# GeoStat-Framework/PyKrige

Measured on NVIDIA H100. Metric: kriged grid points/sec (N data -> M grid), higher is better.
Workload: dtype f64

## Files before the change

include/krige_b200.h:

```cpp
#ifndef KRIGE_B200_H
#define KRIGE_B200_H

#include <stddef.h>
#include <stdint.h>

#ifdef __cplusplus
extern "C" {
#endif

#define KB200_OK            0
#define KB200_EBADARG      -1
#define KB200_EUNSUPPORTED -2
#define KB200_ESINGULAR    -3
#define KB200_ECUDA        -4
#define KB200_ENOMEM       -5
#define KB200_ESTATE       -6

#define KB200_VG_LINEAR       0
#define KB200_VG_POWER        1
#define KB200_VG_GAUSSIAN     2
#define KB200_VG_EXPONENTIAL  3
#define KB200_VG_SPHERICAL    4
#define KB200_VG_HOLE_EFFECT  5
#define KB200_VG_TABLE        6
// ... 97 lines not shown
                            int exact_values, double eps,
                            int n_rl, int n_hd, const double* drift_data);
int kb200_group_set_problem_knn(kb200_group g, int dim, int64_t n,
                                const double* x, const double* y, const double* z,
                                const double* values,
                                const double* center, const double* aniso,
                                int model, const double* vparams, int n_vparams,
                                int exact_values, double eps);
int kb200_group_execute_points(kb200_group g, int64_t m,
                               const double* px, const double* py, const double* pz,
                               const double* drift_pts,
                               double* z_out, double* ss_out);
int kb200_group_execute_grid(kb200_group g,
                             int64_t nx, int64_t ny, int64_t nz,
                             const double* gx, const double* gy, const double* gz,
                             const double* drift_pts,
                             int64_t first, int64_t count,
                             double* z_out, double* ss_out);
int kb200_group_execute_knn_points(kb200_group g, int k, int64_t m,
                                   const double* px, const double* py, const double* pz,
                                   double* z_out, double* ss_out);
int kb200_group_execute_knn_grid(kb200_group g, int k,
                                 int64_t nx, int64_t ny, int64_t nz,
                                 const double* gx, const double* gy, const double* gz,
                                 int64_t first, int64_t count,
                                 double* z_out, double* ss_out);

int kb200_set_coordinates(kb200_handle h, int coordinates_type);

int kb200_set_stream(kb200_handle h, void* cuda_stream);

int  kb200_last_timings(kb200_handle h, double* ms, int n);
void kb200_reset_counters(kb200_handle h);

int kb200_set_variogram_table(kb200_handle h, int64_t n_nodes, double dmax, const double* gamma_nodes);

int kb200_set_pseudo_inverse(kb200_handle h, int enable);

int kb200_set_values(kb200_handle h, int n_fields, int64_t n, const double* values);

int kb200_experimental_variogram(kb200_handle h, int dim, int64_t n,
                                 const double* x, const double* y, const double* z, const double* values,
                                 int nlags, double* counts, double* lag_sum, double* semi_sum, double* dminmax);

int kb200_statistics(kb200_handle h, double* delta, double* sigma);

int kb200_loo(kb200_handle h, double* z, double* sigmasq);
int kb200_knn_loo(kb200_handle h, int k, double* z, double* sigmasq);

int kb200_lgo(kb200_handle h, const int32_t* group, int n_groups, double* z, double* sigmasq);
int kb200_knn_lgo(kb200_handle h, int k, const int32_t* group, int n_groups, double* z, double* sigmasq);

int64_t kb200_debug_fetch(kb200_handle h, int what, double* out, int64_t cap);

#ifdef __cplusplus
}
#endif
#endif
```

pykrige_b200/_cabi.py:

```python
import ctypes
import os
import numpy as np

_HERE = os.path.dirname(os.path.abspath(__file__))
LIB_PATH = os.path.join(_HERE, "libkrige_b200.so")

KB200_OK = 0
KB200_EBADARG = -1
KB200_EUNSUPPORTED = -2
KB200_ESINGULAR = -3
KB200_ECUDA = -4
KB200_ENOMEM = -5
KB200_ESTATE = -6

KB200_F64 = 0
KB200_F32 = 1
KB200_F64X = 2
KB200_F64X5 = 3
KB200_F64X4 = 4
DTYPES = {"float64": KB200_F64, "float32": KB200_F32, "float64x": KB200_F64X, "float64x5": KB200_F64X5,
          "float64x4": KB200_F64X4}
MAX_DRIFT = 15
MAX_FIELDS = 64

EXPORTS = [
    "kb200_create", "kb200_destroy", "kb200_last_error", "kb200_version",
    "kb200_set_problem", "kb200_execute_points", "kb200_execute_grid",
    "kb200_execute_points_dev", "kb200_execute_grid_dev",
    "kb200_execute_knn_points", "kb200_execute_knn_grid", "kb200_execute_knn_grid_dev",
    "kb200_set_problem_knn",
    "kb200_blob_bytes", "kb200_blob_ptr", "kb200_describe_problem", "kb200_blob_commit",
    "kb200_set_coordinates", "kb200_set_stream", "kb200_last_timings", "kb200_reset_counters", "kb200_debug_fetch",
    "kb200_experimental_variogram", "kb200_statistics", "kb200_loo", "kb200_knn_loo", "kb200_lgo", "kb200_knn_lgo",
    "kb200_set_pseudo_inverse",
    "kb200_set_variogram_table", "kb200_set_device_drift", "kb200_set_values",
    "kb200_group_create", "kb200_group_destroy", "kb200_group_last_error", "kb200_group_size", "kb200_group_member",
    "kb200_group_set_problem", "kb200_group_set_problem_knn", "kb200_group_execute_points",
    "kb200_group_execute_grid", "kb200_group_execute_knn_points", "kb200_group_execute_knn_grid",
]

_c_double_p = ctypes.POINTER(ctypes.c_double)
_lib = None


class KrigeB200Error(RuntimeError):
    pass


def load_library():
    global _lib
    if _lib is not None:
        return _lib
    if not os.path.exists(LIB_PATH):
        raise KrigeB200Error(
            "libkrige_b200.so is not built (%s). Run `python -c 'import __graft_entry__ as g; g.build()'` "
            "or `make -C pykrige_b200/csrc`. backend='cuda' has no CPU fallback." % LIB_PATH
        )
    lib = ctypes.CDLL(LIB_PATH)
    h = ctypes.c_void_p
    i64 = ctypes.c_int64
    i32 = ctypes.c_int
    dp = ctypes.c_void_p
    lib.kb200_create.argtypes = [ctypes.POINTER(h), i32]
    lib.kb200_destroy.argtypes = [h]
    lib.kb200_destroy.restype = None
    lib.kb200_last_error.argtypes = [h]
    lib.kb200_last_error.restype = ctypes.c_char_p
    lib.kb200_version.restype = i32
    prob = [h, i32, i32, i64, dp, dp, dp, dp, dp, dp, i32, dp, i32, i32, ctypes.c_double, i32, i32, dp]
    lib.kb200_set_problem.argtypes = prob
    lib.kb200_describe_problem.argtypes = prob
    lib.kb200_set_problem_knn.argtypes = [h, i32, i64, dp, dp, dp, dp, dp, dp, i32, dp, i32, i32, ctypes.c_double]
    lib.kb200_execute_points.argtypes = [h, i64, dp, dp, dp, dp, dp, dp]
    lib.kb200_execute_points_dev.argtypes = [h, i64, dp, dp, dp, dp, dp, dp]
    grid = [h, i64, i64, i64, dp, dp, dp, dp, i64, i64, dp, dp]
    lib.kb200_execute_grid.argtypes = grid
    lib.kb200_execute_grid_dev.argtypes = grid
    lib.kb200_execute_knn_points.argtypes = [h, i32, i64, dp, dp, dp, dp, dp]
    kgrid = [h, i32, i64, i64, i64, dp, dp, dp, i64, i64, dp, dp]
    lib.kb200_execute_knn_grid.argtypes = kgrid
    lib.kb200_execute_knn_grid_dev.argtypes = kgrid
    lib.kb200_blob_bytes.argtypes = [h]
    lib.kb200_blob_bytes.restype = i64
    lib.kb200_blob_ptr.argtypes = [h]
    lib.kb200_blob_ptr.restype = ctypes.c_void_p
    lib.kb200_blob_commit.argtypes = [h]
    lib.kb200_set_coordinates.argtypes = [h, i32]
    lib.kb200_set_stream.argtypes = [h, ctypes.c_void_p]
    lib.kb200_last_timings.argtypes = [h, _c_double_p, i32]
    lib.kb200_reset_counters.argtypes = [h]
    lib.kb200_reset_counters.restype = None
    lib.kb200_debug_fetch.argtypes = [h, i32, dp, i64]
    lib.kb200_debug_fetch.restype = i64
    lib.kb200_experimental_variogram.argtypes = [h, i32, i64, dp, dp, dp, dp, i32, dp, dp, dp, dp]
    lib.kb200_statistics.argtypes = [h, dp, dp]
    lib.kb200_loo.argtypes = [h, dp, dp]
    lib.kb200_knn_loo.argtypes = [h, i32, dp, dp]
    lib.kb200_lgo.argtypes = [h, dp, i32, dp, dp]
    lib.kb200_knn_lgo.argtypes = [h, i32, dp, i32, dp, dp]
    lib.kb200_set_pseudo_inverse.argtypes = [h, i32]
    lib.kb200_set_variogram_table.argtypes = [h, i64, ctypes.c_double, dp]
    lib.kb200_set_device_drift.argtypes = [h, i32, dp, i64, i64, dp, dp, dp]
    lib.kb200_set_values.argtypes = [h, i32, i64, dp]
    lib.kb200_group_create.argtypes = [ctypes.POINTER(h), i32, ctypes.POINTER(i32)]
    lib.kb200_group_destroy.argtypes = [h]
    lib.kb200_group_destroy.restype = None
    lib.kb200_group_last_error.argtypes = [h]
    lib.kb200_group_last_error.restype = ctypes.c_char_p
    lib.kb200_group_size.argtypes = [h]
    lib.kb200_group_member.argtypes = [h, i32]
    lib.kb200_group_member.restype = ctypes.c_void_p
    lib.kb200_group_set_problem.argtypes = prob
    lib.kb200_group_set_problem_knn.argtypes = lib.kb200_set_problem_knn.argtypes
    lib.kb200_group_execute_points.argtypes = lib.kb200_execute_points.argtypes
    lib.kb200_group_execute_grid.argtypes = grid
    lib.kb200_group_execute_knn_points.argtypes = lib.kb200_execute_knn_points.argtypes
    lib.kb200_group_execute_knn_grid.argtypes = kgrid
    _lib = lib
    return lib


_aux = None
_aux_error = None

# ... 184 lines not shown
        self._check(self.lib.kb200_describe_problem(*args))

    def execute_grid_dev(self, nx, ny, nz, d_gx, d_gy, d_gz, d_drift, first, count, d_z, d_ss):
        self._check(self.lib.kb200_execute_grid_dev(self._h, int(nx), int(ny), int(nz), d_gx, d_gy, d_gz, d_drift,
                                                    int(first), int(count), d_z, d_ss))

    def execute_points_dev(self, m, d_px, d_py, d_pz, d_drift, d_z, d_ss):
        self._check(self.lib.kb200_execute_points_dev(self._h, int(m), d_px, d_py, d_pz, d_drift, d_z, d_ss))

    def execute_knn_grid_dev(self, k, nx, ny, nz, d_gx, d_gy, d_gz, first, count, d_z, d_ss):
        self._check(self.lib.kb200_execute_knn_grid_dev(self._h, int(k), int(nx), int(ny), int(nz), d_gx, d_gy, d_gz,
                                                        int(first), int(count), d_z, d_ss), knn=True)

    def blob(self):
        return int(self.lib.kb200_blob_ptr(self._h) or 0), int(self.lib.kb200_blob_bytes(self._h))

    def blob_commit(self):
        self._check(self.lib.kb200_blob_commit(self._h))

    def set_coordinates(self, geographic):
        self._check(self.lib.kb200_set_coordinates(self._h, 1 if geographic else 0))

    def set_stream(self, cuda_stream):
        self._check(self.lib.kb200_set_stream(self._h, ctypes.c_void_p(int(cuda_stream))))

    def timings(self):
        buf = (ctypes.c_double * 12)()
        n = self.lib.kb200_last_timings(self._h, buf, 12)
        return {TIMING_KEYS[i]: buf[i] for i in range(n)}

    def reset_counters(self):
        self.lib.kb200_reset_counters(self._h)

    def set_variogram_table(self, nodes, dmax):
        nodes = _f64(nodes)
        self._check(self.lib.kb200_set_variogram_table(self._h, nodes.size, float(dmax), _ptr(nodes)))

    def set_pseudo_inverse(self, enable):
        self._check(self.lib.kb200_set_pseudo_inverse(self._h, 1 if enable else 0))

    def set_device_drift(self, wells, ext):
        w = _f64(np.asarray(wells, dtype=np.float64).reshape(-1, 3)) if wells is not None and len(wells) else None
        if ext is not None:
            ex, ey, ez = _f64(np.ravel(ext[0])), _f64(np.ravel(ext[1])), _f64(ext[2])
            if ez.shape != (ey.size, ex.size):
                raise ValueError("external drift raster must be shaped (len(y), len(x))")
            args = (ex.size, ey.size, _ptr(ex), _ptr(ey), _ptr(ez))
        else:
            args = (0, 0, None, None, None)
        self._check(self.lib.kb200_set_device_drift(self._h, 0 if w is None else w.shape[0], _ptr(w), *args))

    def set_values(self, fields):
        if fields is None:
            self._check(self.lib.kb200_set_values(self._h, 0, 0, None))
            self.n_fields = 0
            return
        f = np.ascontiguousarray(fields, dtype=np.float64)
        self.n_fields = 0
        self._check(self.lib.kb200_set_values(self._h, int(f.shape[0]), int(f.shape[1]), _ptr(f)))
        self.n_fields = int(f.shape[0])

    def experimental_variogram(self, X, values, nlags, geographic=False):
        X = np.asarray(X, dtype=np.float64)
        dim = X.shape[1]
        cols = [_f64(X[:, c]) for c in range(dim)]
        v = _f64(values)
# ... 92 lines not shown
```

pykrige_b200/csrc/api.cu:

```cuda
#include <cuda_runtime.h>
#include <string>
#include <vector>
#include <cstring>
#include <cstdio>
#include <cmath>
#include <cstdlib>
#include <algorithm>
#include <thread>
#include <climits>
#include "kernels.h"

#define KB_VERSION 2000
static const int64_t KB_STAGE_PTS = 1 << 20;
#define KB_TILE_COST_32 0.607
#define KB_TILE_COST_16 0.403
static const int64_t KB_STAGE_MIN = 1 << 18;
#define KB_TN_FIELDS 32

struct Src {
    bool grid; int64_t nx, ny, nz;
    const double *a, *b, *c;
    int64_t first, count;
    const double* d_drift; int64_t drift_stride, drift_first;

    Src sub(int64_t o, int64_t m) const {
        Src s = *this; s.first += o; s.count = m; s.drift_first += o; return s;
    }
    PointSource point_source() const {
        PointSource ps{};
        ps.grid = grid ? 1 : 0;
        ps.px = a; ps.py = b; ps.pz = c; ps.gx = a; ps.gy = b; ps.gz = c;
        ps.nx = nx; ps.ny = ny; ps.nz = nz; ps.first = first;
        return ps;
    }
};

enum Tm { TM_ASSEMBLE, TM_CHOLESKY, TM_TRTRI, TM_PACK_DUAL, TM_SOLVE, TM_FINALIZE, TM_H2D, TM_D2H, TM_KNN_SEARCH,
          TM_KNN_SOLVE, TM_SOLVE_LAUNCHES, TM_LAUNCHES, TM_COUNT };
enum Ev { EV_UPLOAD, EV_ADJUSTED, EV_ASM, EV_KNN_BUILT = EV_ASM, EV_FACTOR, EV_INVERT, EV_DUAL, EV_PACKED,
          EV_RUN, EV_RUN_END, EV_H2D, EV_H2D_END, EV_D2H_END, EV_COUNT };

struct DevBuf {
    void* p = nullptr; size_t cap = 0;
    cudaError_t reserve(size_t bytes) {
        if (bytes <= cap) return cudaSuccess;
        if (p) cudaFree(p);
        p = nullptr; cap = 0;
        cudaError_t e = cudaMalloc(&p, bytes);
// ... 6 lines not shown

struct kb200_ctx {
    int device = 0;
    cudaStream_t stream = nullptr;
    bool own_stream = false;
    std::string err;

    bool described = false, ready = false, knn_ready = false;
    bool local_factor = false;
    int slices = 0;
    int gform = 0;
    int geo = 0;
    int pinv = 0;
    int pinv_sweeps = 0, pinv_rank = 0;
    int dim = 2, dtype = KB200_F64, n = 0, n_pad = 0, ld = 0, n_rl = 0, n_hd = 0, K1 = 1, na = 2, nrb = 0;
    VgParams vg{};
    Aniso an{};
    DriftScale ds{};
    PackMap pm{};
    std::vector<double> hx, hy, hz, hval, hdrift;
    double bb_lo[3] = {0, 0, 0}, bb_hi[3] = {0, 0, 0};
    int nf = 0; int64_t nf_n = 0;
    std::vector<double> hfields;
    int aux_cols = KB_MAXAUX;
    int64_t zstride = 0;
    int pin_blocks = 0;

    DevBuf blob;
    size_t off_consts = 0, off_ax = 0, off_ay = 0, off_az = 0, off_tiles = 0, off_rowscale = 0, blob_bytes = 0;

    DevBuf wC, wW, wT, wF, wRaw, wFlag;
    DevBuf wPts, wOut, wDrift, wScratch, wFstage;
    int num_sms = 132;
    DeviceDrift dd{};
    DevBuf wWells, wExt;
    int n_dev = 0;
    void* pin[2] = {nullptr, nullptr};
    cudaStream_t copy_stream = nullptr;
    cudaEvent_t evk[2] = {}, evc[2] = {};
    cudaStream_t hi_stream = nullptr;
    std::vector<cudaEvent_t> fev;
    DevBuf kSorted, kCells, kFields;
    DevBuf wVario;
    DevBuf wLoo;
    DevBuf wLgo, wLgoM;
    const int* lgo_sg = nullptr; const int* lgo_qg = nullptr;
    DevBuf wTab;
    std::vector<double> htab;
    double tab_dmax = 0.0; int tab_n = 0;
    KnnParams kp{};
    int k_ncells = 0;

    cudaEvent_t ev[EV_COUNT] = {};
    double tm[TM_COUNT] = {};
    long long launches = 0, solve_launches = 0;
};

static int fail(kb200_ctx* h, int code, const std::string& msg) {
    if (h) h->err = msg;
    return code;
}
#define CU(h, expr) do { cudaError_t _e = (expr); if (_e != cudaSuccess) { \
    return fail(h, _e == cudaErrorMemoryAllocation ? KB200_ENOMEM : KB200_ECUDA, \
                std::string(#expr) + ": " + cudaGetErrorString(_e)); } } while (0)

static size_t align_up(size_t v, size_t a) { return (v + a - 1) / a * a; }
// ... 26 lines not shown
    h->gform = (int)hdr[HDR_GFORM];
    for (int c = 0; c <= KB200_MAX_DRIFT; ++c) { h->ds.shift[c] = hdr[HDR_SHIFT + c]; h->ds.scale[c] = hdr[HDR_SCALE + c]; }
    return true;
}

enum RawCol { RAW_X, RAW_Y, RAW_Z, RAW_V, RAW_DRIFT };
static double* raw_col(const kb200_ctx* h, int c) { return h->wRaw.as<double>() + (size_t)c * h->n; }
static double* kriged_values(const kb200_ctx* h) { return raw_col(h, h->nf ? RAW_DRIFT + h->n_hd : RAW_V); }

enum AuxBlock { AUX_F, AUX_H, AUX_U };
static double* aux_block(const kb200_ctx* h, int i) {
    return h->wF.as<double>() + (size_t)i * h->aux_cols * h->n_pad;
}

extern "C" int kb200_version(void) { return KB_VERSION; }

extern "C" int kb200_create(kb200_handle* out, int device) {
    if (!out) return KB200_EBADARG;
    *out = nullptr;
    int cnt = 0;
    cudaError_t e = cudaGetDeviceCount(&cnt);
    if (e != cudaSuccess || cnt == 0) return KB200_ECUDA;
    kb200_ctx* h = new kb200_ctx();
    if (device < 0) { if (cudaGetDevice(&device) != cudaSuccess) device = 0; }
    if (device >= cnt) { delete h; return KB200_EBADARG; }
    h->device = device;
    if (cudaSetDevice(device) != cudaSuccess) { delete h; return KB200_ECUDA; }
    if (cudaStreamCreateWithFlags(&h->stream, cudaStreamNonBlocking) != cudaSuccess) { delete h; return KB200_ECUDA; }
    h->own_stream = true;
    for (auto& ev : h->ev) if (cudaEventCreate(&ev) != cudaSuccess) { delete h; return KB200_ECUDA; }
    if (kbk_factor_init() != cudaSuccess || kbk_solve_init() != cudaSuccess || kbk_solve_tf32_init() != cudaSuccess ||
        kbk_solve_i8_init() != cudaSuccess || kbk_ev_init() != cudaSuccess || kbk_pinv_init() != cudaSuccess) { delete h; return KB200_ECUDA; }
    if (cudaDeviceGetAttribute(&h->num_sms, cudaDevAttrMultiProcessorCount, device) != cudaSuccess || h->num_sms < 1) h->num_sms = 132;
    *out = h;
    return KB200_OK;
}

extern "C" void kb200_destroy(kb200_handle h) {
    if (!h) return;
    cudaSetDevice(h->device);
    cudaStreamSynchronize(h->stream);
    for (DevBuf* b : {&h->blob, &h->wC, &h->wW, &h->wT, &h->wF, &h->wRaw, &h->wFlag,
                      &h->wPts, &h->wOut, &h->wDrift, &h->wScratch, &h->wFstage, &h->kSorted, &h->kCells, &h->kFields, &h->wVario, &h->wTab,
                      &h->wLoo, &h->wLgo, &h->wLgoM, &h->wWells, &h->wExt}) b->release();
    for (int i = 0; i < 2; ++i) {
        if (h->pin[i]) cudaFreeHost(h->pin[i]);
        if (h->evk[i]) cudaEventDestroy(h->evk[i]);
        if (h->evc[i]) cudaEventDestroy(h->evc[i]);
    }
    if (h->copy_stream) cudaStreamDestroy(h->copy_stream);
    if (h->hi_stream) cudaStreamDestroy(h->hi_stream);
    for (auto& e : h->fev) cudaEventDestroy(e);
    for (auto& ev : h->ev) if (ev) cudaEventDestroy(ev);
    if (h->own_stream && h->stream) cudaStreamDestroy(h->stream);
    delete h;
}

extern "C" const char* kb200_last_error(kb200_handle h) { return h ? h->err.c_str() : "null handle"; }

extern "C" int kb200_set_stream(kb200_handle h, void* s) {
    if (!h) return KB200_EBADARG;
    if (h->own_stream && h->stream) { cudaStreamSynchronize(h->stream); cudaStreamDestroy(h->stream); }
    h->stream = reinterpret_cast<cudaStream_t>(s);
    h->own_stream = false;
    return KB200_OK;
}
// ... 7 lines not shown
    return KB200_OK;
}

extern "C" int kb200_set_pseudo_inverse(kb200_handle h, int enable) {
    if (!h) return KB200_EBADARG;
    h->pinv = enable ? 1 : 0;
    drop_problem(h);
    return KB200_OK;
}

extern "C" int kb200_set_values(kb200_handle h, int n_fields, int64_t n, const double* values) {
    if (!h) return KB200_EBADARG;
    drop_problem(h);
    h->nf = 0; h->nf_n = 0; h->hfields.clear();
    if (n_fields == 0) return KB200_OK;
    if (n_fields < 0 || n_fields > KB200_MAX_FIELDS)
        return fail(h, KB200_EBADARG, "n_fields must be in [0, " + std::to_string(KB200_MAX_FIELDS) + "]");
    if (n < 1 || n > (1LL << 30) || !values) return fail(h, KB200_EBADARG, "values: n >= 1 rows and a non-NULL array");
    const size_t cnt = (size_t)n * n_fields;
    for (size_t i = 0; i < cnt; ++i)
        if (!std::isfinite(values[i]))
            return fail(h, KB200_EBADARG, "values must be finite (field " + std::to_string(i / n) + ", row " +
                        std::to_string(i % n) + ")");
    h->hfields.assign(values, values + cnt);
    h->nf = n_fields; h->nf_n = n;
    return KB200_OK;
}

extern "C" void kb200_reset_counters(kb200_handle h) {
    if (!h) return;
    h->launches = 0; h->solve_launches = 0;
    for (double& t : h->tm) t = 0.0;
}

extern "C" int kb200_last_timings(kb200_handle h, double* ms, int n) {
    if (!h || !ms) return KB200_EBADARG;
    h->tm[TM_SOLVE_LAUNCHES] = (double)h->solve_launches;
    h->tm[TM_LAUNCHES] = (double)h->launches;
    int m = std::min(n, (int)TM_COUNT);
    for (int i = 0; i < m; ++i) ms[i] = h->tm[i];
    return m;
}

static double host_gamma(const kb200_ctx* h, const VgParams& v, double d) {
    switch (v.model) {
        case KB200_VG_LINEAR: return v.p0 * d + v.p1;
        case KB200_VG_POWER: return v.p0 * std::pow(d, v.p1) + v.p2;
        case KB200_VG_TABLE: {
            if (h->tab_n < 2) return 1.0;
            const double inv_h = (h->tab_n - 1) / std::sqrt(h->tab_dmax);
            int last = (int)std::min<double>(h->tab_n - 1, std::ceil(std::sqrt(std::max(d, 0.0)) * inv_h));
            double g = h->htab[0];
            for (int i = 0; i <= last; ++i) g = std::max(g, h->htab[2 * (size_t)i]);
            return g;
        }
        default: return v.p0 + v.p2;
    }
}

extern "C" int kb200_set_variogram_table(kb200_handle h, int64_t n_nodes, double dmax, const double* gamma_nodes) {
    if (!h) return KB200_EBADARG;
    if (n_nodes < 16 || n_nodes > (1LL << 26) || !gamma_nodes || !(dmax > 0.0) || !std::isfinite(dmax))
        return fail(h, KB200_EBADARG, "variogram table: 16 <= n_nodes <= 2^26, dmax > 0");
    const int n = (int)n_nodes;
    for (int i = 0; i < n; ++i)
        if (!std::isfinite(gamma_nodes[i])) return fail(h, KB200_EBADARG, "variogram table: the callable must be finite on [0, dmax] (node " + std::to_string(i) + ")");
// ... 375 lines not shown
    if (ext && (ext_nx < 1 || ext_ny < 1 || ext_nx > (1 << 30) || ext_ny > (1 << 30) || !ext_x || !ext_y || !ext_z))
        return fail(h, KB200_EBADARG, "device drift: bad external_Z raster description");
    drop_problem(h);
    cudaSetDevice(h->device);
    h->dd = DeviceDrift{};
    if (n_wells) {
        CU(h, h->wWells.reserve((size_t)3 * n_wells * 8));
        CU(h, cudaMemcpyAsync(h->wWells.p, wells, (size_t)3 * n_wells * 8, cudaMemcpyHostToDevice, h->stream));
        h->dd.n_wells = n_wells; h->dd.wells = h->wWells.as<double>();
    }
    if (ext) {
        const size_t nx = (size_t)ext_nx, ny = (size_t)ext_ny;
        CU(h, h->wExt.reserve((nx + ny + nx * ny) * 8));
        double* d = h->wExt.as<double>();
        CU(h, cudaMemcpyAsync(d, ext_x, nx * 8, cudaMemcpyHostToDevice, h->stream));
        CU(h, cudaMemcpyAsync(d + nx, ext_y, ny * 8, cudaMemcpyHostToDevice, h->stream));
        CU(h, cudaMemcpyAsync(d + nx + ny, ext_z, nx * ny * 8, cudaMemcpyHostToDevice, h->stream));
        bool sorted = true;
        for (size_t i = 1; i < nx && sorted; ++i) sorted = ext_x[i] >= ext_x[i - 1];
        for (size_t i = 1; i < ny && sorted; ++i) sorted = ext_y[i] >= ext_y[i - 1];
        h->dd.ext = 1; h->dd.ext_nx = (int)ext_nx; h->dd.ext_ny = (int)ext_ny; h->dd.ext_sorted = sorted ? 1 : 0;
        h->dd.ext_x = d; h->dd.ext_y = d + nx; h->dd.ext_z = d + nx + ny;
    }
    CU(h, cudaStreamSynchronize(h->stream));
    return KB200_OK;
}

static int launch_solve(kb200_ctx* h, const Src& s, double* d_z, double* d_ss, int tp) {
    cudaStream_t st = h->stream;
    const BlobView b = blob_view(h);
    const bool i8 = h->slices != 0;
    const bool f32 = h->dtype == KB200_F32;
    long long ntiles = (s.count + tp - 1) / tp;
    int grid = (int)std::min<long long>(ntiles, h->num_sms);
    CU(h, h->wScratch.reserve(i8 ? kbk_solve_i8_scratch_bytes(h->slices, h->n, grid) : f32 ? kbk_solve_tf32_scratch_bytes(h->n, grid)
                                  : kbk_solve_pt_scratch_doubles(h->n, grid) * sizeof(double)));
    SolvePtParams pp{};
    pp.vg = h->vg; pp.an = h->an; pp.ps = s.point_source();
    pp.n = h->n; pp.na = h->na; pp.nrb = h->nrb; pp.n_rl = h->n_rl; pp.n_hd = h->n_hd;
    pp.ax = b.ax; pp.ay = b.ay; pp.az = b.az;
    pp.tiles = b.tiles; pp.pm = h->pm; pp.ds = h->ds;
    pp.consts = b.consts;
    pp.dd = h->dd; pp.n_dev = h->n_dev;
    pp.drift_pts = s.d_drift; pp.drift_stride = s.drift_stride; pp.drift_first = s.drift_first;
    pp.m = s.count; pp.scratch = h->wScratch.as<double>(); pp.gform = h->gform;
    pp.z_out = d_z; pp.ss_out = d_ss;
    pp.nf = h->nf; pp.zstride = h->zstride;
    if (h->nf) {
        CU(h, h->wFstage.reserve((size_t)grid * h->na * tp * sizeof(double)));
        pp.fstage = h->wFstage.as<double>();
    }
    pp.rowscale = b.rowscale;
    if (i8) CU(h, kbk_solve_i8(h->slices, h->dim, pp, grid, st));
    else if (f32) CU(h, kbk_solve_tf32(h->dim, pp, grid, st));
    else CU(h, kbk_solve_pt(h->dim, pp, grid, tp, st));
    h->launches += 1; h->solve_launches += 1;
    return KB200_OK;
}

static double tile_cost(int tp) { return tp == 64 ? 1.0 : (tp == 32 ? KB_TILE_COST_32 : KB_TILE_COST_16); }

static int run_solve(kb200_ctx* h, const Src& s, double* d_z, double* d_ss) {
    const bool i8 = h->slices != 0;
    const bool f32 = h->dtype == KB200_F32;
    if (i8 || f32) return launch_solve(h, s, d_z, d_ss, i8 ? kbk_solve_i8_tile_points() : kbk_solve_tf32_tile_points());
    const long long S = h->num_sms;
    const int TW = h->nf ? KB_TN_FIELDS : KB_TN;
    if (const char* e = std::getenv("KB200_TILE")) {
        const int t = std::min(std::atoi(e), TW);
        if (t == 64 || t == 32 || t == 16) return launch_solve(h, s, d_z, d_ss, t);
    }
    const long long nt64 = (s.count + TW - 1) / TW;
    const long long main_pts = std::min<long long>(s.count, (nt64 / S) * S * TW);
    const long long rem = s.count - main_pts;
    if (main_pts > 0) {
        int rc = launch_solve(h, s.sub(0, main_pts), d_z, d_ss, TW); if (rc) return rc;
    }
    if (rem > 0) {
        int best = TW; double bc = 1e300;
        for (int tp : {64, 32, 16}) {
            if (tp > TW) continue;
            const long long nt = (rem + tp - 1) / tp;
            const double c = (double)((nt + S - 1) / S) * tile_cost(tp);
            if (c < bc * 0.999) { bc = c; best = tp; }
        }
        int rc = launch_solve(h, s.sub(main_pts, rem), d_z + main_pts, d_ss + main_pts, best); if (rc) return rc;
    }
    return KB200_OK;
}

template <class Launch>
static int run_to_host(kb200_ctx* h, int64_t total, double* z_out, double* ss_out, Launch launch) {
    cudaStream_t st = h->stream;
    const int nzb = h->nf ? h->nf : 1;
    h->zstride = total;
    CU(h, h->wOut.reserve((size_t)(nzb + 1) * total * 8));
    double* dz = h->wOut.as<double>();
    double* dss = dz + (size_t)nzb * total;
    CU(h, cudaEventRecord(h->ev[EV_RUN], st));
// ... 878 lines not shown
```

pykrige_b200/csrc/common.cuh:

```cuda
#pragma once
#include <cuda_runtime.h>
#include <stdint.h>
#include <math.h>
#include "../../include/krige_b200.h"

#define KB_WARP 32

#define KB_BM 256
#define KB_TN 64
#define KB_BK 16
#define KB_NB 64
#define KB_MAXAUX (KB200_MAX_DRIFT + 2)
#define KB_MAXRB 128

struct VgParams {
    int model;
    double p0, p1, p2;
    double inv_a;
    double c0;
    double eps;
    int exact;
    const double2* tab;
    double tab_inv_h;
    int tab_n;
// ... 182 lines not shown
                 "selp.u32 %0, 1, 0, p;\n\t}\n"
                 : "=r"(ok) : "r"(kb_smem_u32(bar)), "r"(parity) : "memory");
    return ok != 0;
}
__device__ __forceinline__ void kb_mbar_wait(uint64_t* bar, uint32_t parity) {
    for (uint32_t it = 0; it < (1u << 26); ++it)
        if (kb_mbar_try_wait(bar, parity)) return;
    __trap();
}
__device__ __forceinline__ void kb_fence_publish_async() {
    __threadfence();
    asm volatile("fence.proxy.async.global;\n" ::: "memory");
}
__device__ __forceinline__ void kb_bulk_g2s(void* dst, const void* src, uint32_t bytes, uint64_t* bar) {
    asm volatile("cp.async.bulk.shared::cluster.global.mbarrier::complete_tx::bytes [%0], [%1], %2, [%3];\n"
                 :: "r"(kb_smem_u32(dst)), "l"(src), "r"(bytes), "r"(kb_smem_u32(bar)) : "memory");
}

__device__ __forceinline__ uint64_t kb_policy_evict_last() {
    uint64_t p;
    asm volatile("createpolicy.fractional.L2::evict_last.b64 %0, 1.0;\n" : "=l"(p));
    return p;
}
__device__ __forceinline__ uint64_t kb_policy_evict_first() {
    uint64_t p;
    asm volatile("createpolicy.fractional.L2::evict_first.b64 %0, 1.0;\n" : "=l"(p));
    return p;
}
__device__ __forceinline__ void kb_bulk_g2s_hint(void* dst, const void* src, uint32_t bytes, uint64_t* bar, uint64_t policy) {
    asm volatile("cp.async.bulk.shared::cluster.global.mbarrier::complete_tx::bytes.L2::cache_hint [%0], [%1], %2, [%3], %4;\n"
                 :: "r"(kb_smem_u32(dst)), "l"(src), "r"(bytes), "r"(kb_smem_u32(bar)), "l"(policy) : "memory");
}

__device__ __forceinline__ uint64_t kb_wgmma_desc(uint32_t smem_addr, uint32_t lbo, uint32_t sbo) {
    return (uint64_t)((smem_addr >> 4) & 0x3fffu) | ((uint64_t)((lbo >> 4) & 0x3fffu) << 16) |
           ((uint64_t)((sbo >> 4) & 0x3fffu) << 32);
}
__device__ __forceinline__ void kb_wgmma_fence() { asm volatile("wgmma.fence.sync.aligned;\n" ::: "memory"); }
__device__ __forceinline__ void kb_wgmma_commit() { asm volatile("wgmma.commit_group.sync.aligned;\n" ::: "memory"); }
template <int N>
__device__ __forceinline__ void kb_wgmma_wait() { asm volatile("wgmma.wait_group.sync.aligned %0;\n" :: "n"(N) : "memory"); }
__device__ __forceinline__ void kb_reg_fence(float& r) { asm volatile("" : "+f"(r) :: "memory"); }
__device__ __forceinline__ void kb_reg_fence(uint32_t& r) { asm volatile("" : "+r"(r) :: "memory"); }
__device__ __forceinline__ void kb_named_sync(int id, int threads) {
    asm volatile("bar.sync %0, %1;\n" :: "r"(id), "r"(threads) : "memory");
}

#define KB_CUDA_OK(expr) do { cudaError_t _e = (expr); if (_e != cudaSuccess) return _e; } while (0)
```

pykrige_b200/csrc/kernels.h:

```cpp
#pragma once
#include <type_traits>
#include "common.cuh"

template <int... Vs>
struct KbList {
    template <typename F>
    static cudaError_t dispatch(int v, F&& f) {
        cudaError_t e = cudaErrorInvalidValue;
        (void)((v == Vs && ((e = f(std::integral_constant<int, Vs>{})), true)) || ...);
        return e;
    }
    template <typename F>
    static cudaError_t for_each(F&& f) {
        cudaError_t e = cudaSuccess;
        (void)(((e = f(std::integral_constant<int, Vs>{})) == cudaSuccess) && ...);
        return e;
    }
};
using KbDims = KbList<2, 3, KB_GEO>;
using KbModels = KbList<KB200_VG_LINEAR, KB200_VG_POWER, KB200_VG_GAUSSIAN, KB200_VG_EXPONENTIAL, KB200_VG_SPHERICAL,
                        KB200_VG_HOLE_EFFECT, KB200_VG_TABLE>;
using KbSlices = KbList<4, 5, 6>;
using KbBools = KbList<0, 1>;

// ... 153 lines not shown
        muphi += mu * phi[a];
    }
    P.ss_out[pj] = P.vg.c0 - q + rmu;
    P.z_out[pj] = zc - muphi;
}
#endif

cudaError_t kbk_adjust_data(int dim, const Aniso& an, int n, const double* x, const double* y, const double* z,
                            double* ax, double* ay, double* az, cudaStream_t st);
cudaError_t kbk_assemble(int dim, const VgParams& vg, int n, int n_pad, int ld,
                         const double* ax, const double* ay, const double* az, double* C, cudaStream_t st);
cudaError_t kbk_cholesky(double* C, double* W, double* Lstage, int ld, int n_pad, int* flag, double dtol, cudaStream_t st,
                         cudaStream_t hi, cudaEvent_t* ev, int n_ev, int* launches);
cudaError_t kbk_trtri(const double* L, double* W, double* T1, int ld, int n_pad, cudaStream_t st, int* launches);
cudaError_t kbk_dual(const double* W, int ld, int n, int n_pad, int n_rl, int n_hd, int nv,
                     const double* ax, const double* ay, const double* az, const DriftScale& ds,
                     const double* hd, const double* values,
                     double* Fz, double* Hz, double* Uz, double* consts, int* flag, cudaStream_t st, int* launches);
cudaError_t kbk_pack(const double* W, int ld, int n, int n_pad, int na, const double* Uz,
                     const PackMap& pm, void* out, cudaStream_t st);

size_t      kbk_general_inverse_workspace_bytes(int n_pad);
cudaError_t kbk_general_inverse(double* C, int ld, int n_pad, void* work, int* flag, double ptol,
                                cudaStream_t st, int* launches);
cudaError_t kbk_dual_gform(const double* G, int ld, int n, int n_pad, int n_rl, int n_hd, int nv,
                           const double* ax, const double* ay, const double* az, const DriftScale& ds,
                           const double* hd, const double* values,
                           double* Fz, double* Uz, double* consts, int* flag, cudaStream_t st, int* launches);
cudaError_t kbk_pack_gform(const double* G, int ld, int n, int n_pad, int na, const double* Uz,
                           const PackMap& pm, void* out, cudaStream_t st);
cudaError_t kbk_factor_init();
cudaError_t kbk_solve_init();
cudaError_t kbk_solve_pt(int dim, const SolvePtParams& p, int grid, int tile_points , cudaStream_t st);
size_t      kbk_solve_pt_scratch_doubles(int n, int grid);

cudaError_t kbk_solve_tf32_init();
cudaError_t kbk_solve_tf32(int dim, const SolvePtParams& p, int grid, cudaStream_t st);
cudaError_t kbk_pack_tf32(const double* W, int ld, int n, int n_pad, int na, const double* Uz, const PackMap& pm,
                          void* out, cudaStream_t st);
size_t      kbk_solve_tf32_scratch_bytes(int n, int grid);
int         kbk_solve_tf32_tile_points();

bool        kbk_i8_valid_slices(int S);
cudaError_t kbk_solve_i8_init();
cudaError_t kbk_solve_i8(int S, int dim, const SolvePtParams& p, int grid, cudaStream_t st);
cudaError_t kbk_pack_i8(int S, const double* W, int ld, int n, int n_pad, int na, const double* Uz,
                        int* rowexp, double* rowscale, const long long* tile_off_dev, void* out, cudaStream_t st);
int         kbk_i8_nrb(int S, int n, int na);
int         kbk_i8_rows(int S, int n, int na);
long long   kbk_i8_total_tiles(int S, int n, int na, long long* tile_off);
size_t      kbk_i8_tile_bytes(int S);
size_t      kbk_solve_i8_scratch_bytes(int S, int n, int grid);
int         kbk_solve_i8_tile_points();

struct KnnParams {
    VgParams vg;
    Aniso an;
    PointSource ps;
    int dim, n, k;
    const double* ax; const double* ay; const double* az; const double* values;
    const int* sorig;
    int gx, gy, gz;
    int r0;
    double ox, oy, oz, inv_cell, cell;
    const int* cell_start;
    long long m;
// ... 90 lines not shown
```

pykrige_b200/csrc/solve.cu:

```cuda
#include "common.cuh"
#include "kernels.h"

#define PT_STAGES 5
#define PT_THREADS 384
#define PT_CONS0 (PT_THREADS / 32 - 8)
#define PT_STAGE_BYTES ((KB_BM * KB_BK + KB_BK * KB_TN) * 8)

template <int C>
__device__ __forceinline__ void pt_reduce_scatter_step(double* v, int lane, int mask) {
    if constexpr (C >= 2) {
        const bool up = (lane & mask) != 0;
#pragma unroll
        for (int h = 0; h < C / 2; ++h) {
            const double send = up ? v[h] : v[h + C / 2];
            const double keep = up ? v[h + C / 2] : v[h];
            v[h] = keep + __shfl_xor_sync(0xffffffffu, send, mask);
        }
    } else {
        v[0] += __shfl_xor_sync(0xffffffffu, v[0], mask);
    }
}
template <int CNT>
__device__ __forceinline__ void pt_reduce_scatter(double* v, int lane) {
    pt_reduce_scatter_step<CNT>(v, lane, 16);
    pt_reduce_scatter_step<(CNT >= 2 ? CNT / 2 : 1)>(v, lane, 8);
    pt_reduce_scatter_step<(CNT >= 4 ? CNT / 4 : 1)>(v, lane, 4);
}
template <int CNT>
__device__ __forceinline__ int pt_reduce_scatter_index(int i, int lane) {
    int o = i, c = CNT;
    for (int mask = 16; mask >= 4; mask >>= 1) {
        if (c >= 2) { c /= 2; if (lane & mask) o += c; }
        else if (lane & mask) return -1;
    }
    return o;
}

template <int DIM, int MODEL, int NT, bool FIELDS>
__global__ void __launch_bounds__(PT_THREADS, 1) solve_kernel_pt(const __grid_constant__ SolvePtParams P) {
    constexpr int TN = NT * 8;
    extern __shared__ __align__(128) unsigned char smem_raw[];
    double* Ts = reinterpret_cast<double*>(smem_raw);
    double* Bs = Ts + PT_STAGES * KB_BM * KB_BK;
    double* qred = Bs + PT_STAGES * KB_BK * TN;
    double* auxs = qred + 8 * TN;
    uint64_t* full = reinterpret_cast<uint64_t*>(auxs + KB_MAXAUX * TN);
    uint64_t* empty = full + PT_STAGES;

    const int tid = threadIdx.x, lane = tid & 31, warp = tid >> 5;
    const int nk = (P.n + KB_BK - 1) / KB_BK;
    double* scratch = P.scratch + (size_t)blockIdx.x * nk * (KB_BK * TN);
    const double* gt = reinterpret_cast<const double*>(P.tiles);
    const long long ntiles = (P.m + TN - 1) / TN;

    if (tid == 0) {
        for (int s = 0; s < PT_STAGES; ++s) { kb_mbar_init(&full[s], 1); kb_mbar_init(&empty[s], 8); }
        kb_fence_mbar_init();
    }
    __syncthreads();

    const uint32_t stages_per_tile = (uint32_t)(P.pm.tile_off[P.nrb - 1] + P.pm.ktiles[P.nrb - 1]);
    const int cw = warp - PT_CONS0;

    for (uint32_t it = 0; blockIdx.x + (long long)it * gridDim.x < ntiles; ++it) {
        const long long tile = blockIdx.x + (long long)it * gridDim.x;
        const uint32_t git = it * stages_per_tile;
        {
            const int pl = tid % TN;
            const int ks = tid / TN;
            const long long pj = tile * TN + pl;
            const bool pvalid = pj < P.m;
            double px = 0.0, py = 0.0, pz = 0.0;
            if (pvalid) kb_load_point<DIM>(P.ps, P.an, pj, px, py, pz);
            for (int t = ks; t < nk; t += PT_THREADS / TN) {
                double* bt = scratch + (size_t)t * (KB_BK * TN);
#pragma unroll
                for (int k4 = 0; k4 < 4; ++k4) {
                    double v[4];
#pragma unroll
                    for (int kk = 0; kk < 4; ++kk) {
                        const int k = t * KB_BK + k4 * 4 + kk;
                        double val = 0.0;
                        if (pvalid && k < P.n) {
                            double d = kb_dist<DIM>(__ldg(P.ax + k), __ldg(P.ay + k), KB_HASZ(DIM) ? __ldg(P.az + k) : 0.0,
                                                    px, py, pz);
                            val = kb_cov_rhs<MODEL>(P.vg, d);
                        }
                        v[kk] = val;
                    }
                    double2* dst = reinterpret_cast<double2*>(bt + (k4 * NT + (pl >> 3)) * 32 + (pl & 7) * 4);
                    dst[0] = make_double2(v[0], v[1]);
                    dst[1] = make_double2(v[2], v[3]);
                }
            }
            kb_fence_publish_async();
        }
        __syncthreads();

        if (warp == 0) {
            if (lane == 0) {
                uint32_t g = git;
                const uint64_t pol_w = kb_policy_evict_last(), pol_c = kb_policy_evict_first();
                long long tau = 0;
                for (int I = 0; I < P.nrb; ++I) {
                    const int kt = P.pm.ktiles[I];
                    for (int t = 0; t < kt; ++t, ++tau, ++g) {
                        const int s = g % PT_STAGES;
                        kb_mbar_wait(&empty[s], (uint32_t)(((g / PT_STAGES) & 1) ^ 1));
                        kb_mbar_expect_tx(&full[s], (KB_BM * KB_BK + KB_BK * TN) * 8);
                        kb_bulk_g2s_hint(Ts + (size_t)s * KB_BM * KB_BK, gt + (size_t)tau * (KB_BM * KB_BK),
                                         KB_BM * KB_BK * 8, &full[s], pol_w);
                        kb_bulk_g2s_hint(Bs + (size_t)s * KB_BK * TN, scratch + (size_t)t * (KB_BK * TN),
                                         KB_BK * TN * 8, &full[s], pol_c);
                    }
                }
            }
        } else if (warp >= PT_CONS0) {
            uint32_t g = git;
            constexpr int QV = NT >= 4 ? NT / 4 : 1;
            double* qrow = qred + cw * TN;
#pragma unroll
            for (int v = 0; v < QV; ++v) {
                const int o = pt_reduce_scatter_index<2 * NT>(v, lane);
                if (o >= 0) qrow[(o >> 1) * 8 + 2 * (lane & 3) + (o & 1)] = 0.0;
            }
            const int mtl[2] = {cw, 15 - cw};
            for (int I = 0; I < P.nrb; ++I) {
                const uint32_t gend = g + (uint32_t)P.pm.ktiles[I];
                uint32_t glim[2];
#pragma unroll
                for (int q = 0; q < 2; ++q) {
                    const int r0 = I * KB_BM + mtl[q] * 16;
                    if (r0 + 15 >= P.n && r0 < P.n + P.na) glim[q] = gend;
                    else if (r0 >= P.n + P.na) glim[q] = g;
                    else glim[q] = g + (uint32_t)(r0 / KB_BK + 1);
                }
                double acc[2][NT][4];
#pragma unroll
                for (int a = 0; a < 2; ++a)
#pragma unroll
                    for (int b = 0; b < NT; ++b)
#pragma unroll
                        for (int i = 0; i < 4; ++i) acc[a][b][i] = 0.0;
                for (; g < gend; ++g) {
                    const int s = g % PT_STAGES;
                    kb_mbar_wait(&full[s], (uint32_t)((g / PT_STAGES) & 1));
                    const bool on0 = g < glim[0], on1 = g < glim[1];
                    if (on0 || on1) {
                        const double2* ts = reinterpret_cast<const double2*>(Ts + (size_t)s * KB_BM * KB_BK);
                        const double* bs = Bs + (size_t)s * KB_BK * TN;
#pragma unroll
                        for (int k4 = 0; k4 < 4; ++k4) {
                            double fa[2][2];
#pragma unroll
                            for (int q = 0; q < 2; ++q) {
                                const double2 v = ts[(mtl[q] * 4 + k4) * 32 + lane];
                                fa[q][0] = v.x; fa[q][1] = v.y;
                            }
#pragma unroll
                            for (int nt = 0; nt < NT; ++nt) {
                                const double fb = bs[(k4 * NT + nt) * 32 + lane];
                                if (on0) kb_dmma_16x8x4(acc[0][nt], fa[0], fb);
                                if (on1) kb_dmma_16x8x4(acc[1][nt], fa[1], fb);
                            }
                        }
                    }
                    __syncwarp();
                    if (lane == 0) kb_mbar_arrive(&empty[s]);
                }
#pragma unroll
                for (int q = 0; q < 2; ++q)
#pragma unroll
                    for (int h = 0; h < 2; ++h) {
                        const int r = I * KB_BM + mtl[q] * 16 + 8 * h + (lane >> 2);
                        if (r < P.n) {
                            if (!P.gform) {
#pragma unroll
                                for (int nt = 0; nt < NT; ++nt)
#pragma unroll
                                    for (int i = 0; i < 2; ++i) acc[q][nt][2 * h + i] *= acc[q][nt][2 * h + i];
                            } else {
                                const double* bt = P.scratch + ((size_t)blockIdx.x * nk + (r >> 4)) * (KB_BK * TN) +
                                                   ((r & 15) >> 2) * (NT * 32) + (r & 3);
#pragma unroll
                                for (int nt = 0; nt < NT; ++nt)
#pragma unroll
                                    for (int i = 0; i < 2; ++i) {
                                        const int c = nt * 8 + 2 * (lane & 3) + i;
                                        acc[q][nt][2 * h + i] *= bt[(c >> 3) * 32 + (c & 7) * 4];
                                    }
                            }
                        } else {
                            if (r < P.n + P.na) {
                                double* ao = (FIELDS ? P.fstage + (int)(blockIdx.x * P.na * TN) : auxs) + (r - P.n) * TN +
                                             2 * (lane & 3);
#pragma unroll
                                for (int nt = 0; nt < NT; ++nt) {
                                    ao[nt * 8] = acc[q][nt][2 * h];
                                    ao[nt * 8 + 1] = acc[q][nt][2 * h + 1];
                                }
                            }
// ... 1 lines not shown
                            for (int nt = 0; nt < NT; ++nt) { acc[q][nt][2 * h] = 0.0; acc[q][nt][2 * h + 1] = 0.0; }
                        }
                    }
                double part[2 * NT];
#pragma unroll
                for (int nt = 0; nt < NT; ++nt)
#pragma unroll
                    for (int i = 0; i < 2; ++i)
                        part[2 * nt + i] = ((acc[0][nt][i] + acc[0][nt][2 + i]) + acc[1][nt][i]) + acc[1][nt][2 + i];
                pt_reduce_scatter<2 * NT>(part, lane);
#pragma unroll
                for (int v = 0; v < QV; ++v) {
                    const int o = pt_reduce_scatter_index<2 * NT>(v, lane);
                    if (o >= 0) qrow[(o >> 1) * 8 + 2 * (lane & 3) + (o & 1)] += part[v];
                }
            }
        }
        __syncthreads();

        if (tid < TN) {
            const long long pj = tile * TN + tid;
            if (pj < P.m) {
                double q = 0.0;
#pragma unroll
                for (int w = 0; w < 8; ++w) q += qred[w * TN + tid];
                if constexpr (FIELDS)
                    kb_finalize_point<DIM, double, true>(P, pj, q, P.fstage + (int)(blockIdx.x * P.na * TN) + tid, TN);
                else
                    kb_finalize_point<DIM, double>(P, pj, q, auxs + tid, TN);
            }
        }
        __syncthreads();
    }
}

static size_t solve_smem_pt() {
    return (size_t)PT_STAGES * (KB_BM * KB_BK + KB_BK * KB_TN) * sizeof(double) + 8 * KB_TN * sizeof(double) +
           KB_MAXAUX * KB_TN * sizeof(double) + 2 * PT_STAGES * sizeof(uint64_t) + 64;
}
size_t kbk_solve_pt_scratch_doubles(int n, int grid) {
    return (size_t)grid * ((n + KB_BK - 1) / KB_BK) * (KB_BK * KB_TN);
}


using PtWidths = KbList<16, 32, 64>;

cudaError_t kbk_solve_init() {
    const int sm = (int)solve_smem_pt();
    return KbDims::for_each([&](auto D) {
        return KbModels::for_each([&](auto M) {
            return PtWidths::for_each([&](auto TN) {
                KB_CUDA_OK(cudaFuncSetAttribute(solve_kernel_pt<D, M, TN / 8, false>,
                                                cudaFuncAttributeMaxDynamicSharedMemorySize, sm));
                if constexpr (TN == 64) return cudaSuccess;
                else return cudaFuncSetAttribute(solve_kernel_pt<D, M, TN / 8, true>,
                                                 cudaFuncAttributeMaxDynamicSharedMemorySize, sm);
            });
        });
    });
}

cudaError_t kbk_solve_pt(int dim, const SolvePtParams& p, int grid, int tile_points, cudaStream_t st) {
    const size_t sm = solve_smem_pt();
    return KbDims::dispatch(dim, [&](auto D) {
        return KbModels::dispatch(p.vg.model, [&](auto M) {
            return PtWidths::dispatch(tile_points, [&](auto TN) {
                if (!p.nf) solve_kernel_pt<D, M, TN / 8, false><<<grid, PT_THREADS, sm, st>>>(p);
                else if constexpr (TN == 64) return cudaErrorInvalidValue;
                else solve_kernel_pt<D, M, TN / 8, true><<<grid, PT_THREADS, sm, st>>>(p);
                return cudaGetLastError();
            });
        });
    });
}
```

Before: 1.767 million.

## Multicast shared factor tiles across 2-CTA clusters in f64 point solve

The f64 point-solve kernel now launches as 2-CTA thread-block clusters. Each CTA bulk-loads half of the shared factor tile and multicasts it to both CTAs, which roughly halves global/L2 traffic for the factor operand. The empty barriers now take arrivals from consumers in both CTAs, the tile loop is paired so both CTAs in a cluster run the same number of iterations, and the grid is sized from the maximum number of active clusters, with the tile-cost constants retuned. In exchange the two CTAs are lock-stepped through cross-CTA barrier arrivals, and the grid is limited by cluster occupancy, which could leave some SMs idle.

```diff
diff --git a/include/krige_b200.h b/include/krige_b200.h
--- a/include/krige_b200.h
+++ b/include/krige_b200.h
@@ -153,6 +153,7 @@
 
 int  kb200_last_timings(kb200_handle h, double* ms, int n);
 void kb200_reset_counters(kb200_handle h);
+int  kb200_solve_round(kb200_handle h);
 
 int kb200_set_variogram_table(kb200_handle h, int64_t n_nodes, double dmax, const double* gamma_nodes);
 
diff --git a/pykrige_b200/_cabi.py b/pykrige_b200/_cabi.py
--- a/pykrige_b200/_cabi.py
+++ b/pykrige_b200/_cabi.py
@@ -30,7 +30,7 @@
     "kb200_execute_knn_points", "kb200_execute_knn_grid", "kb200_execute_knn_grid_dev",
     "kb200_set_problem_knn",
     "kb200_blob_bytes", "kb200_blob_ptr", "kb200_describe_problem", "kb200_blob_commit",
-    "kb200_set_coordinates", "kb200_set_stream", "kb200_last_timings", "kb200_reset_counters", "kb200_debug_fetch",
+    "kb200_set_coordinates", "kb200_set_stream", "kb200_last_timings", "kb200_reset_counters", "kb200_solve_round", "kb200_debug_fetch",
     "kb200_experimental_variogram", "kb200_statistics", "kb200_loo", "kb200_knn_loo", "kb200_lgo", "kb200_knn_lgo",
     "kb200_set_pseudo_inverse",
     "kb200_set_variogram_table", "kb200_set_device_drift", "kb200_set_values",
@@ -90,6 +90,8 @@
     lib.kb200_last_timings.argtypes = [h, _c_double_p, i32]
     lib.kb200_reset_counters.argtypes = [h]
     lib.kb200_reset_counters.restype = None
+    lib.kb200_solve_round.argtypes = [h]
+    lib.kb200_solve_round.restype = ctypes.c_int
     lib.kb200_debug_fetch.argtypes = [h, i32, dp, i64]
     lib.kb200_debug_fetch.restype = i64
     lib.kb200_experimental_variogram.argtypes = [h, i32, i64, dp, dp, dp, dp, i32, dp, dp, dp, dp]
@@ -340,6 +342,9 @@
     def reset_counters(self):
         self.lib.kb200_reset_counters(self._h)
 
+    def solve_round(self):
+        return self.lib.kb200_solve_round(self._h)
+
     def set_variogram_table(self, nodes, dmax):
         nodes = _f64(nodes)
         self._check(self.lib.kb200_set_variogram_table(self._h, nodes.size, float(dmax), _ptr(nodes)))
diff --git a/pykrige_b200/csrc/api.cu b/pykrige_b200/csrc/api.cu
--- a/pykrige_b200/csrc/api.cu
+++ b/pykrige_b200/csrc/api.cu
@@ -12,8 +12,8 @@
 
 #define KB_VERSION 2000
 static const int64_t KB_STAGE_PTS = 1 << 20;
-#define KB_TILE_COST_32 0.607
-#define KB_TILE_COST_16 0.403
+#define KB_TILE_COST_32 0.576
+#define KB_TILE_COST_16 0.354
 static const int64_t KB_STAGE_MIN = 1 << 18;
 #define KB_TN_FIELDS 32
 
@@ -86,6 +86,7 @@
     DevBuf wC, wW, wT, wF, wRaw, wFlag;
     DevBuf wPts, wOut, wDrift, wScratch, wFstage;
     int num_sms = 132;
+    int pt_clusters = 66;
     DeviceDrift dd{};
     DevBuf wWells, wExt;
     int n_dev = 0;
@@ -178,6 +179,7 @@
     if (kbk_factor_init() != cudaSuccess || kbk_solve_init() != cudaSuccess || kbk_solve_tf32_init() != cudaSuccess ||
         kbk_solve_i8_init() != cudaSuccess || kbk_ev_init() != cudaSuccess || kbk_pinv_init() != cudaSuccess) { delete h; return KB200_ECUDA; }
     if (cudaDeviceGetAttribute(&h->num_sms, cudaDevAttrMultiProcessorCount, device) != cudaSuccess || h->num_sms < 1) h->num_sms = 132;
+    if (kbk_solve_pt_max_clusters(&h->pt_clusters) != cudaSuccess || h->pt_clusters < 1) { delete h; return KB200_ECUDA; }
     *out = h;
     return KB200_OK;
 }
@@ -251,6 +253,8 @@
     h->launches = 0; h->solve_launches = 0;
     for (double& t : h->tm) t = 0.0;
 }
+
+extern "C" int kb200_solve_round(kb200_handle h) { return h ? 2 * h->pt_clusters : KB200_EBADARG; }
 
 extern "C" int kb200_last_timings(kb200_handle h, double* ms, int n) {
     if (!h || !ms) return KB200_EBADARG;
@@ -692,7 +696,8 @@
     const bool i8 = h->slices != 0;
     const bool f32 = h->dtype == KB200_F32;
     long long ntiles = (s.count + tp - 1) / tp;
-    int grid = (int)std::min<long long>(ntiles, h->num_sms);
+    int grid = (i8 || f32) ? (int)std::min<long long>(ntiles, h->num_sms)
+                           : (int)std::min<long long>((ntiles + 1) / 2 * 2, 2LL * h->pt_clusters);
     CU(h, h->wScratch.reserve(i8 ? kbk_solve_i8_scratch_bytes(h->slices, h->n, grid) : f32 ? kbk_solve_tf32_scratch_bytes(h->n, grid)
                                   : kbk_solve_pt_scratch_doubles(h->n, grid) * sizeof(double)));
     SolvePtParams pp{};
@@ -724,7 +729,7 @@
     const bool i8 = h->slices != 0;
     const bool f32 = h->dtype == KB200_F32;
     if (i8 || f32) return launch_solve(h, s, d_z, d_ss, i8 ? kbk_solve_i8_tile_points() : kbk_solve_tf32_tile_points());
-    const long long S = h->num_sms;
+    const long long S = 2LL * h->pt_clusters;
     const int TW = h->nf ? KB_TN_FIELDS : KB_TN;
     if (const char* e = std::getenv("KB200_TILE")) {
         const int t = std::min(std::atoi(e), TW);
diff --git a/pykrige_b200/csrc/common.cuh b/pykrige_b200/csrc/common.cuh
--- a/pykrige_b200/csrc/common.cuh
+++ b/pykrige_b200/csrc/common.cuh
@@ -238,6 +238,31 @@
                  :: "r"(kb_smem_u32(dst)), "l"(src), "r"(bytes), "r"(kb_smem_u32(bar)), "l"(policy) : "memory");
 }
 
+__device__ __forceinline__ uint32_t kb_cluster_ctarank() {
+    uint32_t r;
+    asm volatile("mov.u32 %0, %%cluster_ctarank;\n" : "=r"(r));
+    return r;
+}
+__device__ __forceinline__ uint32_t kb_mapa(const void* p, uint32_t rank) {
+    uint32_t r;
+    asm volatile("mapa.shared::cluster.u32 %0, %1, %2;\n" : "=r"(r) : "r"(kb_smem_u32(p)), "r"(rank));
+    return r;
+}
+__device__ __forceinline__ void kb_cluster_sync() {
+    asm volatile("barrier.cluster.arrive.release.aligned;\n\t"
+                 "barrier.cluster.wait.acquire.aligned;\n" ::: "memory");
+}
+__device__ __forceinline__ void kb_mbar_arrive_cluster(uint32_t bar) {
+    asm volatile("mbarrier.arrive.shared::cluster.b64 _, [%0];\n" :: "r"(bar) : "memory");
+}
+__device__ __forceinline__ void kb_bulk_g2s_multicast_hint(void* dst, const void* src, uint32_t bytes, uint64_t* bar,
+                                                           uint16_t cta_mask, uint64_t policy) {
+    asm volatile("cp.async.bulk.shared::cluster.global.mbarrier::complete_tx::bytes.multicast::cluster.L2::cache_hint"
+                 " [%0], [%1], %2, [%3], %4, %5;\n"
+                 :: "r"(kb_smem_u32(dst)), "l"(src), "r"(bytes), "r"(kb_smem_u32(bar)), "h"(cta_mask), "l"(policy)
+                 : "memory");
+}
+
 __device__ __forceinline__ uint64_t kb_wgmma_desc(uint32_t smem_addr, uint32_t lbo, uint32_t sbo) {
     return (uint64_t)((smem_addr >> 4) & 0x3fffu) | ((uint64_t)((lbo >> 4) & 0x3fffu) << 16) |
            ((uint64_t)((sbo >> 4) & 0x3fffu) << 32);
diff --git a/pykrige_b200/csrc/kernels.h b/pykrige_b200/csrc/kernels.h
--- a/pykrige_b200/csrc/kernels.h
+++ b/pykrige_b200/csrc/kernels.h
@@ -209,6 +209,7 @@
 cudaError_t kbk_factor_init();
 cudaError_t kbk_solve_init();
 cudaError_t kbk_solve_pt(int dim, const SolvePtParams& p, int grid, int tile_points , cudaStream_t st);
+cudaError_t kbk_solve_pt_max_clusters(int* clusters);
 size_t      kbk_solve_pt_scratch_doubles(int n, int grid);
 
 cudaError_t kbk_solve_tf32_init();
diff --git a/pykrige_b200/csrc/solve.cu b/pykrige_b200/csrc/solve.cu
--- a/pykrige_b200/csrc/solve.cu
+++ b/pykrige_b200/csrc/solve.cu
@@ -37,7 +37,7 @@
 }
 
 template <int DIM, int MODEL, int NT, bool FIELDS>
-__global__ void __launch_bounds__(PT_THREADS, 1) solve_kernel_pt(const __grid_constant__ SolvePtParams P) {
+__global__ void __cluster_dims__(2, 1, 1) __launch_bounds__(PT_THREADS, 1) solve_kernel_pt(const __grid_constant__ SolvePtParams P) {
     constexpr int TN = NT * 8;
     extern __shared__ __align__(128) unsigned char smem_raw[];
     double* Ts = reinterpret_cast<double*>(smem_raw);
@@ -54,15 +54,15 @@
     const long long ntiles = (P.m + TN - 1) / TN;
 
     if (tid == 0) {
-        for (int s = 0; s < PT_STAGES; ++s) { kb_mbar_init(&full[s], 1); kb_mbar_init(&empty[s], 8); }
+        for (int s = 0; s < PT_STAGES; ++s) { kb_mbar_init(&full[s], 1); kb_mbar_init(&empty[s], 16); }
         kb_fence_mbar_init();
     }
-    __syncthreads();
+    kb_cluster_sync();
 
     const uint32_t stages_per_tile = (uint32_t)(P.pm.tile_off[P.nrb - 1] + P.pm.ktiles[P.nrb - 1]);
     const int cw = warp - PT_CONS0;
 
-    for (uint32_t it = 0; blockIdx.x + (long long)it * gridDim.x < ntiles; ++it) {
+    for (uint32_t it = 0; (blockIdx.x & ~1u) + (long long)it * gridDim.x < ntiles; ++it) {
         const long long tile = blockIdx.x + (long long)it * gridDim.x;
         const uint32_t git = it * stages_per_tile;
         {
@@ -101,6 +101,8 @@
             if (lane == 0) {
                 uint32_t g = git;
                 const uint64_t pol_w = kb_policy_evict_last(), pol_c = kb_policy_evict_first();
+                constexpr int HALF = KB_BM * KB_BK / 2;
+                const uint32_t rank = kb_cluster_ctarank();
                 long long tau = 0;
                 for (int I = 0; I < P.nrb; ++I) {
                     const int kt = P.pm.ktiles[I];
@@ -108,8 +110,9 @@
                         const int s = g % PT_STAGES;
                         kb_mbar_wait(&empty[s], (uint32_t)(((g / PT_STAGES) & 1) ^ 1));
                         kb_mbar_expect_tx(&full[s], (KB_BM * KB_BK + KB_BK * TN) * 8);
-                        kb_bulk_g2s_hint(Ts + (size_t)s * KB_BM * KB_BK, gt + (size_t)tau * (KB_BM * KB_BK),
-                                         KB_BM * KB_BK * 8, &full[s], pol_w);
+                        kb_bulk_g2s_multicast_hint(Ts + (size_t)s * KB_BM * KB_BK + rank * HALF,
+                                                   gt + (size_t)tau * (KB_BM * KB_BK) + rank * HALF, HALF * 8, &full[s],
+                                                   0x3, pol_w);
                         kb_bulk_g2s_hint(Bs + (size_t)s * KB_BK * TN, scratch + (size_t)t * (KB_BK * TN),
                                          KB_BK * TN * 8, &full[s], pol_c);
                     }
@@ -166,7 +169,10 @@
                         }
                     }
                     __syncwarp();
-                    if (lane == 0) kb_mbar_arrive(&empty[s]);
+                    if (lane == 0) {
+                        kb_mbar_arrive_cluster(kb_smem_u32(&empty[s]));
+                        kb_mbar_arrive_cluster(kb_mapa(&empty[s], kb_cluster_ctarank() ^ 1));
+                    }
                 }
 #pragma unroll
                 for (int q = 0; q < 2; ++q)
@@ -234,6 +240,7 @@
         }
         __syncthreads();
     }
+    kb_cluster_sync();
 }
 
 static size_t solve_smem_pt() {
@@ -262,6 +269,14 @@
     });
 }
 
+cudaError_t kbk_solve_pt_max_clusters(int* clusters) {
+    cudaLaunchConfig_t cfg{};
+    cfg.gridDim = dim3(2);
+    cfg.blockDim = dim3(PT_THREADS);
+    cfg.dynamicSmemBytes = solve_smem_pt();
+    return cudaOccupancyMaxActiveClusters(clusters, solve_kernel_pt<2, KB200_VG_EXPONENTIAL, 8, false>, &cfg);
+}
+
 cudaError_t kbk_solve_pt(int dim, const SolvePtParams& p, int grid, int tile_points, cudaStream_t st) {
     const size_t sm = solve_smem_pt();
     return KbDims::dispatch(dim, [&](auto D) {
```

Result: faster. 1.790 million (median of 6 runs) (+1.3%).
